# vinits5/learning3d

Hardware: AMD Instinct MI355X
Metric: clouds/sec DGCNN-fwd+Chamfer B=32 N=1024; kNN HBM GB/s vs peak at 1/2/4/8 GPU (higher is better)
Workload: dtype f32 (shared-MLP GEMMs as f16x2: fp32 operands carried as an fp16 high part + an fp16 residual (unscaled between the EdgeConv kernel and conv5, 2^12-scaled elsewhere), 3 fp16 MFMA products per fp32 product, f32 accumulate, fp32-level error -- tests bound it by 2x the fp32-MFMA kernel's own error agai

## Files before the change

learning3d_amd/csrc/chamfer.hip:

```cpp
#include "common.h"

#define CTILE 2048
#define CWAVES 4
#define CUNROLL 8
#ifndef CH_SMALL_TILE
#define CH_SMALL_TILE 0
#endif
#define CHAMFER_LL_BLOCKS 64
#define CHAMFER_LL_WS_BYTES (16 + CHAMFER_LL_BLOCKS * 16)

template <int QPL>
__global__ __launch_bounds__(64 * CWAVES) void chamfer_fwd_kernel(const float *__restrict__ xyz1,
                                                                  const float *__restrict__ xyz2, int N,
                                                                  int M, float *__restrict__ dist1,
                                                                  float *__restrict__ dist2,
                                                                  int32_t *__restrict__ idx1,
                                                                  int32_t *__restrict__ idx2)
{
    __shared__ float4 cand[CTILE];
    __shared__ float rbest[CWAVES][QPL][64];
    __shared__ int rbesti[CWAVES][QPL][64];
    const int tid = threadIdx.x, lane = tid & 63, wave = tid >> 6;
    const int b = blockIdx.y;
    const int dir = blockIdx.z;
    const float *qs = dir == 0 ? xyz1 : xyz2;
    const float *cs = dir == 0 ? xyz2 : xyz1;
    const int Nq = dir == 0 ? N : M;
    const int Nc = dir == 0 ? M : N;
    float *dout = dir == 0 ? dist1 : dist2;
    int32_t *iout = dir == 0 ? idx1 : idx2;
    const int q0 = blockIdx.x * (64 * QPL);
    if (q0 >= Nq) return;

    float qx[QPL], qy[QPL], qz[QPL], best[QPL];
    int besti[QPL];
#pragma unroll
    for (int u = 0; u < QPL; u++) {
        int q = min(q0 + u * 64 + lane, Nq - 1);
        const float *p = qs + ((size_t)b * Nq + q) * 3;
        qx[u] = p[0]; qy[u] = p[1]; qz[u] = p[2];
        best[u] = INFINITY; besti[u] = 0x7fffffff;
    }
    const float *cbase = cs + (size_t)b * Nc * 3;
    for (int c0 = 0; c0 < Nc; c0 += CTILE) {
        const int tn = min(CTILE, Nc - c0);
        __syncthreads();
        l3d_stage_points<8>(cbase + (size_t)c0 * 3, tn, tid, 64 * CWAVES, [&](int t, float x, float y, float z) { cand[t] = make_float4(x, y, z, 0.f); });
        __syncthreads();
        const int per = (tn + CWAVES - 1) / CWAVES;
        const int t0 = wave * per, t1 = min(tn, t0 + per);
        int t = t0;
        for (; t + CUNROLL <= t1; t += CUNROLL) {
            float4 c[CUNROLL];
#pragma unroll
            for (int v = 0; v < CUNROLL; v++) c[v] = cand[t + v];
#pragma unroll
            for (int v = 0; v < CUNROLL; v++)
#pragma unroll
                for (int u = 0; u < QPL; u++) {
                    const float dx = c[v].x - qx[u], dy = c[v].y - qy[u], dz = c[v].z - qz[u];
                    const float d = (dx * dx + dy * dy) + dz * dz;
                    const bool lt = d < best[u];
                    best[u] = lt ? d : best[u];
                    besti[u] = lt ? c0 + t + v : besti[u];
                }
        }
        for (; t < t1; t++) {
            const float4 c = cand[t];
#pragma unroll
            for (int u = 0; u < QPL; u++) {
                const float dx = c.x - qx[u], dy = c.y - qy[u], dz = c.z - qz[u];
                const float d = (dx * dx + dy * dy) + dz * dz;
                const bool lt = d < best[u];
                best[u] = lt ? d : best[u];
                besti[u] = lt ? c0 + t : besti[u];
            }
        }
    }
#pragma unroll
    for (int u = 0; u < QPL; u++) { rbest[wave][u][lane] = best[u]; rbesti[wave][u][lane] = besti[u]; }
    __syncthreads();
    if (wave == 0) {
#pragma unroll
        for (int u = 0; u < QPL; u++) {
            float bv = rbest[0][u][lane];
            int bi = rbesti[0][u][lane];
#pragma unroll
            for (int w = 1; w < CWAVES; w++) {
                const float ov = rbest[w][u][lane];
                const int oi = rbesti[w][u][lane];
                const bool take = ov < bv || (ov == bv && oi < bi);
                bv = take ? ov : bv;
                bi = take ? oi : bi;
            }
            const int q = q0 + u * 64 + lane;
            if (q < Nq) {
                dout[(size_t)b * Nq + q] = bv;
                iout[(size_t)b * Nq + q] = bi == 0x7fffffff ? 0 : bi;
            }
        }
    }
}

__device__ __forceinline__ void chamfer_loss_tail(double sq, unsigned *__restrict__ ws, double *__restrict__ partial,
                                                  float *__restrict__ loss, int N, int M)
{
    const int lane = threadIdx.x & 63;
    for (int off = 32; off > 0; off >>= 1) sq += __shfl_down(sq, off, 64);
    double *slots = (double *)(ws + 4);
    const unsigned per_dir = gridDim.x * gridDim.y, total = 2 * per_dir;
    const unsigned slot = (blockIdx.z * gridDim.y + blockIdx.y) * gridDim.x + blockIdx.x;
    unsigned ticket = 0;
    if (lane == 0) {
        __hip_atomic_store(&slots[slot], sq, __ATOMIC_RELAXED, __HIP_MEMORY_SCOPE_AGENT);
        asm volatile("s_waitcnt vmcnt(0)" ::: "memory");
        ticket = __hip_atomic_fetch_add(ws, 1u, __ATOMIC_RELAXED, __HIP_MEMORY_SCOPE_AGENT);
    }
    ticket = __builtin_amdgcn_readfirstlane(ticket);
    if (ticket != total - 1) return;
    double t[2];
#pragma unroll
    for (int z = 0; z < 2; z++) {
        double a = 0.0;
        for (unsigned i = lane; i < per_dir; i += 64) a += __hip_atomic_load(&slots[z * per_dir + i], __ATOMIC_RELAXED, __HIP_MEMORY_SCOPE_AGENT);
        for (int off = 32; off > 0; off >>= 1) a += __shfl_down(a, off, 64);
        t[z] = a;
    }
    if (lane == 0) {
        const double n1 = (double)gridDim.y * N, n2 = (double)gridDim.y * M;
        partial[0] = t[0]; partial[1] = t[1]; partial[2] = n1; partial[3] = n2;
        loss[0] = (float)((t[0] / n1 + t[1] / n2) / 2.0);
        __hip_atomic_store(ws, 0u, __ATOMIC_RELAXED, __HIP_MEMORY_SCOPE_AGENT);
    }
}


template <bool LOSS, int PTILE>
__global__ __launch_bounds__(64 * CWAVES) void chamfer_fwd_packed_kernel(const float *__restrict__ xyz1,
                                                                         const float *__restrict__ xyz2, int N, int M,
                                                                         float *__restrict__ dist1,
                                                                         float *__restrict__ dist2,
                                                                         int32_t *__restrict__ idx1,
                                                                         int32_t *__restrict__ idx2,
                                                                         unsigned *__restrict__ ws, double *__restrict__ partial,
                                                                         float *__restrict__ loss)
{
    typedef float f32x2 __attribute__((ext_vector_type(2)));
    __shared__ float4 cand[PTILE];
    __shared__ float rbest[CWAVES][2][64];
    __shared__ int rbesti[CWAVES][2][64];
    const int tid = threadIdx.x, lane = tid & 63, wave = tid >> 6;
    const int b = blockIdx.y;
    const int dir = blockIdx.z;
    const float *qs = dir == 0 ? xyz1 : xyz2;
    const float *cs = dir == 0 ? xyz2 : xyz1;
    const int Nq = dir == 0 ? N : M;
    const int Nc = dir == 0 ? M : N;
    float *dout = dir == 0 ? dist1 : dist2;
    int32_t *iout = dir == 0 ? idx1 : idx2;
    const int q0 = blockIdx.x * 128;
    if (!LOSS && q0 >= Nq) return;
    if (LOSS && q0 >= Nq) {
        if (wave == 0) chamfer_loss_tail(0.0, ws, partial, loss, N, M);
        return;
    }

    f32x2 qx, qy, qz;
    {
        const float *p0 = qs + ((size_t)b * Nq + min(q0 + lane, Nq - 1)) * 3;
        const float *p1 = qs + ((size_t)b * Nq + min(q0 + 64 + lane, Nq - 1)) * 3;
        qx = f32x2{p0[0], p1[0]}; qy = f32x2{p0[1], p1[1]}; qz = f32x2{p0[2], p1[2]};
    }
    float best0 = INFINITY, best1 = INFINITY;
    int base0 = 0x7fffffff, base1 = 0x7fffffff;
    const float *cbase = cs + (size_t)b * Nc * 3;
    for (int c0 = 0; c0 < Nc; c0 += PTILE) {
        const int tn = min(PTILE, Nc - c0);
        __syncthreads();
        {
            constexpr int NS = PTILE / (64 * CWAVES);
            float sx[NS], sy[NS], sz[NS];
#pragma unroll
            for (int i = 0; i < NS; i++) {
                const float *cp = cbase + (size_t)(c0 + min(tid + i * 64 * CWAVES, tn - 1)) * 3;
                sx[i] = cp[0]; sy[i] = cp[1]; sz[i] = cp[2];
            }
#pragma unroll
            for (int i = 0; i < NS; i++) {
                const int t = tid + i * 64 * CWAVES;
                if (t < tn) cand[t] = make_float4(sx[i], sy[i], sz[i], 0.f);
            }
        }
        __syncthreads();
        const int per = (tn + CWAVES - 1) / CWAVES;
        const int t0 = wave * per, t1 = min(tn, t0 + per);
        int t = t0;
        for (; t + 8 <= t1; t += 8) {
            float4 c[8];
#pragma unroll
            for (int v = 0; v < 8; v++) c[v] = cand[t + v];
            f32x2 d[8];
#pragma unroll
            for (int v = 0; v < 8; v++) {
                const f32x2 dx = f32x2{c[v].x, c[v].x} - qx, dy = f32x2{c[v].y, c[v].y} - qy, dz = f32x2{c[v].z, c[v].z} - qz;
                d[v] = (dx * dx + dy * dy) + dz * dz;
            }
            float m0 = fminf(fminf(d[0][0], d[1][0]), d[2][0]), m1 = fminf(fminf(d[0][1], d[1][1]), d[2][1]);
            m0 = fminf(fminf(m0, d[3][0]), d[4][0]); m1 = fminf(fminf(m1, d[3][1]), d[4][1]);
            m0 = fminf(fminf(m0, d[5][0]), d[6][0]); m1 = fminf(fminf(m1, d[5][1]), d[6][1]);
            m0 = fminf(m0, d[7][0]); m1 = fminf(m1, d[7][1]);
            const bool lt0 = m0 < best0, lt1 = m1 < best1;
            best0 = lt0 ? m0 : best0; base0 = lt0 ? c0 + t : base0;
            best1 = lt1 ? m1 : best1; base1 = lt1 ? c0 + t : base1;
        }
        for (; t < t1; t++) {
            const float4 c = cand[t];
            const f32x2 dx = f32x2{c.x, c.x} - qx, dy = f32x2{c.y, c.y} - qy, dz = f32x2{c.z, c.z} - qz;
            const f32x2 d = (dx * dx + dy * dy) + dz * dz;
            const bool lt0 = d[0] < best0, lt1 = d[1] < best1;
            best0 = lt0 ? d[0] : best0; base0 = lt0 ? c0 + t : base0;
            best1 = lt1 ? d[1] : best1; base1 = lt1 ? c0 + t : base1;
        }
    }
    int bi0 = base0, bi1 = base1;
    {
        bool f0 = base0 == 0x7fffffff, f1 = base1 == 0x7fffffff;
#pragma unroll
        for (int v = 0; v < 8; v++) {
            const int j0 = min(base0 == 0x7fffffff ? 0 : base0 + v, Nc - 1), j1 = min(base1 == 0x7fffffff ? 0 : base1 + v, Nc - 1);
            const float *pa = cbase + (size_t)j0 * 3, *pb = cbase + (size_t)j1 * 3;
            const f32x2 dx = f32x2{pa[0], pb[0]} - qx, dy = f32x2{pa[1], pb[1]} - qy, dz = f32x2{pa[2], pb[2]} - qz;
            const f32x2 d = (dx * dx + dy * dy) + dz * dz;
            if (!f0 && d[0] == best0) { bi0 = j0; f0 = true; }
            if (!f1 && d[1] == best1) { bi1 = j1; f1 = true; }
        }
    }
    rbest[wave][0][lane] = best0; rbesti[wave][0][lane] = bi0;
    rbest[wave][1][lane] = best1; rbesti[wave][1][lane] = bi1;
    __syncthreads();
    if (wave == 0) {
        double sq = 0.0;
#pragma unroll
        for (int u = 0; u < 2; u++) {
            float bv = rbest[0][u][lane];
            int bi = rbesti[0][u][lane];
#pragma unroll
            for (int w = 1; w < CWAVES; w++) {
                const float ov = rbest[w][u][lane];
                const int oi = rbesti[w][u][lane];
                const bool take = ov < bv || (ov == bv && oi < bi);
                bv = take ? ov : bv;
                bi = take ? oi : bi;
            }
            const int q = q0 + u * 64 + lane;
            if (q < Nq) {
                dout[(size_t)b * Nq + q] = bv;
                iout[(size_t)b * Nq + q] = bi == 0x7fffffff ? 0 : bi;
                if (LOSS) sq += (double)sqrtf(bv);
            }
        }
        if (LOSS) chamfer_loss_tail(sq, ws, partial, loss, N, M);
    }
}

int l3d_chamfer_forward_mfma(const float *xyz1, const float *xyz2, int B, int N, int M, float *dist1, float *dist2,
                             int32_t *idx1, int32_t *idx2, hipStream_t stream);

extern "C" int l3d_chamfer_forward_variant(const float *xyz1, const float *xyz2, int B, int N, int M,
                                           float *dist1, float *dist2, int32_t *idx1, int32_t *idx2,
                                           int variant, l3d_stream_t stream)
{
    L3D_REQUIRE(xyz1 && xyz2 && dist1 && dist2 && idx1 && idx2 && B > 0 && N > 0 && M > 0 && variant >= 0 && variant <= 3);
    L3D_REQUIRE(B <= 65535);
    const int l3d_chamfer_forward_mode = variant;
    const int mx = N > M ? N : M;
    if (variant == 3 || (variant == 1 && (long)N * M >= (1L << 24) && (long)2 * l3d_divup(mx, 512) * B >= 128))
        return l3d_chamfer_forward_mfma(xyz1, xyz2, B, N, M, dist1, dist2, idx1, idx2, (hipStream_t)stream);
    const long wgs2 = (long)l3d_divup(mx, 128) * B * 2;
    if (l3d_chamfer_forward_mode == 2 || (l3d_chamfer_forward_mode == 1 && wgs2 * CWAVES >= 1024)) {
        dim3 grid(l3d_divup(mx, 128), B, 2);
        if (mx <= 1024 && CH_SMALL_TILE)
            hipLaunchKernelGGL((chamfer_fwd_packed_kernel<false, 1024>), grid, dim3(64 * CWAVES), 0, (hipStream_t)stream, xyz1, xyz2, N, M,
                               dist1, dist2, idx1, idx2, (unsigned *)nullptr, (double *)nullptr, (float *)nullptr);
        else
            hipLaunchKernelGGL((chamfer_fwd_packed_kernel<false, CTILE>), grid, dim3(64 * CWAVES), 0, (hipStream_t)stream, xyz1, xyz2, N, M,
                               dist1, dist2, idx1, idx2, (unsigned *)nullptr, (double *)nullptr, (float *)nullptr);
    } else if (wgs2 * 2 >= 8192) {
        dim3 grid(l3d_divup(mx, 128), B, 2);
        hipLaunchKernelGGL(chamfer_fwd_kernel<2>, grid, dim3(64 * CWAVES), 0, (hipStream_t)stream, xyz1,
                           xyz2, N, M, dist1, dist2, idx1, idx2);
    } else {
        dim3 grid(l3d_divup(mx, 64), B, 2);
        hipLaunchKernelGGL(chamfer_fwd_kernel<1>, grid, dim3(64 * CWAVES), 0, (hipStream_t)stream, xyz1,
                           xyz2, N, M, dist1, dist2, idx1, idx2);
    }
    return l3d_check_launch();
}

extern "C" int l3d_chamfer_forward(const float *xyz1, const float *xyz2, int B, int N, int M,
                                   float *dist1, float *dist2, int32_t *idx1, int32_t *idx2,
                                   l3d_stream_t stream)
{
    return l3d_chamfer_forward_variant(xyz1, xyz2, B, N, M, dist1, dist2, idx1, idx2, 1, stream);
}

extern "C" int l3d_chamfer_loss_local_mb(const float *dist1, const float *dist2, int B, int N, int M, void *ws, double *partial, float *loss,
                                         l3d_stream_t stream);

extern "C" size_t l3d_chamfer_forward_loss_ws_bytes(int B, int N, int M)
{
    if (B <= 0 || N <= 0 || M <= 0) return 0;
    const size_t fused = 16 + (size_t)2 * B * l3d_divup(N > M ? N : M, 128) * sizeof(double);
    return fused > CHAMFER_LL_WS_BYTES ? fused : CHAMFER_LL_WS_BYTES;
}

extern "C" int l3d_chamfer_forward_loss(const float *xyz1, const float *xyz2, int B, int N, int M, float *dist1, float *dist2,
                                        int32_t *idx1, int32_t *idx2, void *ws, double *partial, float *loss, l3d_stream_t stream)
{
    L3D_REQUIRE(xyz1 && xyz2 && dist1 && dist2 && idx1 && idx2 && ws && partial && loss && B > 0 && N > 0 && M > 0);
    L3D_REQUIRE(B <= 65535);
    const int mx = N > M ? N : M;
    const long wgs2 = (long)l3d_divup(mx, 128) * B * 2;
    if ((long)N * M < (1L << 24) && wgs2 * CWAVES >= 1024) {
        dim3 grid(l3d_divup(mx, 128), B, 2);
        if (mx <= 1024 && CH_SMALL_TILE)
            hipLaunchKernelGGL((chamfer_fwd_packed_kernel<true, 1024>), grid, dim3(64 * CWAVES), 0, (hipStream_t)stream, xyz1, xyz2, N, M, dist1,
                               dist2, idx1, idx2, (unsigned *)ws, partial, loss);
        else
            hipLaunchKernelGGL((chamfer_fwd_packed_kernel<true, CTILE>), grid, dim3(64 * CWAVES), 0, (hipStream_t)stream, xyz1, xyz2, N, M, dist1,
                               dist2, idx1, idx2, (unsigned *)ws, partial, loss);
        return l3d_check_launch();
    }
    const int rc = l3d_chamfer_forward_variant(xyz1, xyz2, B, N, M, dist1, dist2, idx1, idx2, 1, stream);
    return rc ? rc : l3d_chamfer_loss_local_mb(dist1, dist2, B, N, M, ws, partial, loss, stream);
}

#define BTILE 4096
__global__ __launch_bounds__(64) void chamfer_bwd_kernel(const float *__restrict__ xyz1,
                                                         const float *__restrict__ xyz2, int N,
                                                         int M, const float *__restrict__ gd1,
                                                         const float *__restrict__ gd2,
                                                         const int32_t *__restrict__ idx1,
                                                         const int32_t *__restrict__ idx2,
                                                         float *__restrict__ g1,
                                                         float *__restrict__ g2)
{
    __shared__ int32_t sel[BTILE];
    const int lane = threadIdx.x;
    const int b = blockIdx.y;
    const int which = blockIdx.z;
    const float *A = which == 0 ? xyz1 : xyz2;
    const float *C = which == 0 ? xyz2 : xyz1;
    const int NA = which == 0 ? N : M;
    const int NC = which == 0 ? M : N;
    const float *gdA = which == 0 ? gd1 : gd2;
    const float *gdC = which == 0 ? gd2 : gd1;
    const int32_t *ia = which == 0 ? idx1 : idx2;
    const int32_t *ic = which == 0 ? idx2 : idx1;
    float *gout = which == 0 ? g1 : g2;
    if (blockIdx.x * 64 >= NA) return;
    const int i = blockIdx.x * 64 + lane;
    const bool valid = i < NA;
    const int iq = valid ? i : NA - 1;
    const float *ap = A + ((size_t)b * NA + iq) * 3;
    const float ax = ap[0], ay = ap[1], az = ap[2];
    const int j2 = ia[(size_t)b * NA + iq];
    const float *cp = C + ((size_t)b * NC + j2) * 3;
    const float g = gdA[(size_t)b * NA + iq] * 2;
    const float dxd = g * (ax - cp[0]), dyd = g * (ay - cp[1]), dzd = g * (az - cp[2]);
    float gx = 0.f, gy = 0.f, gz = 0.f;
    if (which == 0) { gx += dxd; gy += dyd; gz += dzd; }
    const int32_t *icb = ic + (size_t)b * NC;
    for (int c0 = 0; c0 < NC; c0 += BTILE) {
        const int tn = min(BTILE, NC - c0);
        __syncthreads();
        for (int t = lane; t < tn; t += 64) sel[t] = icb[c0 + t];
        __syncthreads();
        for (int g0 = 0; g0 < tn; g0 += 32) {
            unsigned mask = 0;
            const int gn = min(32, tn - g0);
            if (gn == 32) {
#pragma unroll
                for (int u = 0; u < 32; u++) mask |= sel[g0 + u] == iq ? (1u << u) : 0u;
            } else {
                for (int u = 0; u < gn; u++) mask |= sel[g0 + u] == iq ? (1u << u) : 0u;
            }
#pragma unroll 1
            while (__any(mask != 0)) {
                if (mask != 0) {
                    const int j = c0 + g0 + __builtin_ctz(mask);
                    mask &= mask - 1;
                    const float *pj = C + ((size_t)b * NC + j) * 3;
                    const float gj = gdC[(size_t)b * NC + j] * 2;
                    gx -= gj * (pj[0] - ax);
                    gy -= gj * (pj[1] - ay);
                    gz -= gj * (pj[2] - az);
                }
            }
        }
    }
    if (which == 1) { gx += dxd; gy += dyd; gz += dzd; }
    if (valid) {
        float *o = gout + ((size_t)b * NA + i) * 3;
        o[0] = gx; o[1] = gy; o[2] = gz;
    }
}

#define CB_SORT_MAX 32768
__global__ __launch_bounds__(1024) void chamfer_bwd_sorted_kernel(const float *__restrict__ xyz1,
                                                                  const float *__restrict__ xyz2, int N, int M,
                                                                  const float *__restrict__ gd1,
                                                                  const float *__restrict__ gd2,
                                                                  const int32_t *__restrict__ idx1,
                                                                  const int32_t *__restrict__ idx2,
                                                                  float *__restrict__ g1, float *__restrict__ g2,
                                                                  int P1, int P2, int shift1, int shift2)
{
    extern __shared__ uint32_t keys[];
    const int tid = threadIdx.x;
    const int b = blockIdx.x;
    const int which = blockIdx.y;
    const float *A = which == 0 ? xyz1 : xyz2;
    const float *C = which == 0 ? xyz2 : xyz1;
    const int NA = which == 0 ? N : M;
    const int NC = which == 0 ? M : N;
    const int P = which == 0 ? P2 : P1;
    const int shift = which == 0 ? shift2 : shift1;
    const float *gdA = (which == 0 ? gd1 : gd2) + (size_t)b * NA;
    const float *gdC = (which == 0 ? gd2 : gd1) + (size_t)b * NC;
    const int32_t *ia = (which == 0 ? idx1 : idx2) + (size_t)b * NA;
    const int32_t *ic = (which == 0 ? idx2 : idx1) + (size_t)b * NC;
    float *gout = (which == 0 ? g1 : g2) + (size_t)b * NA * 3;
    const float *Ab = A + (size_t)b * NA * 3, *Cb = C + (size_t)b * NC * 3;

    for (int t = tid; t < P; t += 1024) keys[t] = t < NC ? ((uint32_t)ic[t] << shift) | (uint32_t)t : 0xffffffffu;
    __syncthreads();
    for (int k = 2; k <= P; k <<= 1) {
        for (int j = k >> 1; j > 0; j >>= 1) {
            for (int t = tid; t < (P >> 1); t += 1024) {
                const int lo = ((t & ~(j - 1)) << 1) | (t & (j - 1)), hi = lo | j;
                const uint32_t x = keys[lo], y = keys[hi];
                const bool up = (lo & k) == 0;
                if ((x > y) == up) { keys[lo] = y; keys[hi] = x; }
            }
            __syncthreads();
        }
    }
    const uint32_t jmask = (1u << shift) - 1u;
    for (int i = tid; i < NA; i += 1024) {
        const float ax = Ab[i * 3], ay = Ab[i * 3 + 1], az = Ab[i * 3 + 2];
        const int j2 = ia[i];
        const float g = gdA[i] * 2;
        const float dxd = g * (ax - Cb[j2 * 3]), dyd = g * (ay - Cb[j2 * 3 + 1]), dzd = g * (az - Cb[j2 * 3 + 2]);
        float gx = 0.f, gy = 0.f, gz = 0.f;
        if (which == 0) { gx += dxd; gy += dyd; gz += dzd; }
        const uint32_t want = (uint32_t)i << shift;
        int lo = 0, hi = NC;
        while (lo < hi) {
            const int mid = (lo + hi) >> 1;
            if (keys[mid] < want) lo = mid + 1; else hi = mid;
        }
        for (int pos = lo; pos < NC; pos++) {
            const uint32_t key = keys[pos];
            if ((key >> shift) != (uint32_t)i) break;
            const int j = (int)(key & jmask);
            const float gj = gdC[j] * 2;
            gx -= gj * (Cb[j * 3] - ax);
            gy -= gj * (Cb[j * 3 + 1] - ay);
            gz -= gj * (Cb[j * 3 + 2] - az);
        }
        if (which == 1) { gx += dxd; gy += dyd; gz += dzd; }
        gout[i * 3] = gx; gout[i * 3 + 1] = gy; gout[i * 3 + 2] = gz;
    }
}

extern "C" int l3d_chamfer_backward_variant(const float *xyz1, const float *xyz2, int B, int N, int M,
                                            const float *graddist1, const float *graddist2,
                                            const int32_t *idx1, const int32_t *idx2, float *gradxyz1,
                                            float *gradxyz2, int variant, l3d_stream_t stream)
{
    L3D_REQUIRE(xyz1 && xyz2 && graddist1 && graddist2 && idx1 && idx2 && gradxyz1 && gradxyz2 &&
                B > 0 && N > 0 && M > 0 && variant >= 0 && variant <= 2);
    const int mx = N > M ? N : M;
    const bool sortable = mx <= CB_SORT_MAX;
    if (variant == 2 && !sortable) return L3D_ERR_UNSUPPORTED;
    if (variant != 0 && sortable) {
        int P1 = 2, P2 = 2, s1 = 1, s2 = 1;
        while (P1 < N) { P1 <<= 1; s1++; }
        while (P2 < M) { P2 <<= 1; s2++; }
        const size_t lds = sizeof(uint32_t) * (size_t)(P1 > P2 ? P1 : P2);
        hipLaunchKernelGGL(chamfer_bwd_sorted_kernel, dim3(B, 2), dim3(1024), lds, (hipStream_t)stream, xyz1, xyz2, N, M,
                           graddist1, graddist2, idx1, idx2, gradxyz1, gradxyz2, P1, P2, s1, s2);
        const int rc = l3d_check_launch();
        if (rc == L3D_OK || variant == 2) return rc;
    }
    dim3 grid(l3d_divup(mx, 64), B, 2);
    hipLaunchKernelGGL(chamfer_bwd_kernel, grid, dim3(64), 0, (hipStream_t)stream, xyz1, xyz2, N, M,
                       graddist1, graddist2, idx1, idx2, gradxyz1, gradxyz2);
    return l3d_check_launch();
}

extern "C" int l3d_chamfer_backward(const float *xyz1, const float *xyz2, int B, int N, int M,
                                    const float *graddist1, const float *graddist2,
                                    const int32_t *idx1, const int32_t *idx2, float *gradxyz1,
                                    float *gradxyz2, l3d_stream_t stream)
{
    return l3d_chamfer_backward_variant(xyz1, xyz2, B, N, M, graddist1, graddist2, idx1, idx2, gradxyz1, gradxyz2, 1, stream);
}

__global__ __launch_bounds__(1024) void sqrt_sum_kernel(const float *__restrict__ d1, size_t n1,
                                                        const float *__restrict__ d2, size_t n2,
                                                        double *__restrict__ partial)
{
    __shared__ double part[16];
    const int which = blockIdx.x;
    const float *d = which == 0 ? d1 : d2;
    const size_t n = which == 0 ? n1 : n2;
    double acc = 0.0;
    const size_t n4 = n >> 2;
    for (size_t i = threadIdx.x; i < n4; i += blockDim.x) {
        const float4 v = ((const float4 *)d)[i];
        acc += ((double)sqrtf(v.x) + (double)sqrtf(v.y)) + ((double)sqrtf(v.z) + (double)sqrtf(v.w));
    }
    for (size_t i = (n4 << 2) + threadIdx.x; i < n; i += blockDim.x) acc += (double)sqrtf(d[i]);
    for (int off = 32; off > 0; off >>= 1) acc += __shfl_down(acc, off, 64);
    if ((threadIdx.x & 63) == 0) part[threadIdx.x >> 6] = acc;
    __syncthreads();
    if (threadIdx.x == 0) {
        double t = 0.0;
        for (int w = 0; w < 16; w++) t += part[w];
        partial[which] = t;
        partial[2 + which] = (double)n;
    }
}

extern "C" int l3d_chamfer_partials(const float *dist1, const float *dist2, int B, int N, int M,
                                    double *partial, l3d_stream_t stream)
{
    L3D_REQUIRE(dist1 && dist2 && partial && B > 0 && N > 0 && M > 0);
    hipLaunchKernelGGL(sqrt_sum_kernel, dim3(2), dim3(1024), 0, (hipStream_t)stream, dist1,
                       (size_t)B * N, dist2, (size_t)B * M, partial);
    return l3d_check_launch();
}

__global__ __launch_bounds__(256) void chamfer_loss_local_mb_kernel(const float *__restrict__ d1, size_t n1,
                                                                    const float *__restrict__ d2, size_t n2,
                                                                    unsigned *__restrict__ ws, double *__restrict__ partial,
                                                                    float *__restrict__ loss)
{
    __shared__ double part[2][4];
    __shared__ bool last;
    double acc1 = 0.0, acc2 = 0.0;
    const size_t a4 = n1 >> 2, b4 = n2 >> 2, m4 = a4 > b4 ? a4 : b4;
    const size_t stride = (size_t)gridDim.x * 256;
    for (size_t i = (size_t)blockIdx.x * 256 + threadIdx.x; i < m4; i += stride) {
        if (i < a4) {
            const float4 v = ((const float4 *)d1)[i];
            acc1 += ((double)sqrtf(v.x) + (double)sqrtf(v.y)) + ((double)sqrtf(v.z) + (double)sqrtf(v.w));
        }
        if (i < b4) {
            const float4 v = ((const float4 *)d2)[i];
            acc2 += ((double)sqrtf(v.x) + (double)sqrtf(v.y)) + ((double)sqrtf(v.z) + (double)sqrtf(v.w));
        }
    }
    if (blockIdx.x == 0) {
        for (size_t i = (a4 << 2) + threadIdx.x; i < n1; i += 256) acc1 += (double)sqrtf(d1[i]);
        for (size_t i = (b4 << 2) + threadIdx.x; i < n2; i += 256) acc2 += (double)sqrtf(d2[i]);
    }
    for (int off = 32; off > 0; off >>= 1) { acc1 += __shfl_down(acc1, off, 64); acc2 += __shfl_down(acc2, off, 64); }
    if ((threadIdx.x & 63) == 0) { part[0][threadIdx.x >> 6] = acc1; part[1][threadIdx.x >> 6] = acc2; }
    __syncthreads();
    double *slots = (double *)(ws + 4);
    if (threadIdx.x == 0) {
        slots[2 * blockIdx.x] = (part[0][0] + part[0][1]) + (part[0][2] + part[0][3]);
        slots[2 * blockIdx.x + 1] = (part[1][0] + part[1][1]) + (part[1][2] + part[1][3]);
        __threadfence();
        last = atomicAdd(ws, 1u) == gridDim.x - 1;
    }
    __syncthreads();
    if (last && threadIdx.x < 64) {
        __threadfence();
        double t1 = 0.0, t2 = 0.0;
        if (threadIdx.x < gridDim.x) {
            t1 = __builtin_nontemporal_load(&slots[2 * threadIdx.x]);
            t2 = __builtin_nontemporal_load(&slots[2 * threadIdx.x + 1]);
        }
        for (int off = 32; off > 0; off >>= 1) { t1 += __shfl_down(t1, off, 64); t2 += __shfl_down(t2, off, 64); }
        if (threadIdx.x == 0) {
            partial[0] = t1; partial[1] = t2; partial[2] = (double)n1; partial[3] = (double)n2;
            loss[0] = (float)((t1 / (double)n1 + t2 / (double)n2) / 2.0);
            ws[0] = 0;
        }
    }
}

extern "C" size_t l3d_chamfer_loss_local_ws_bytes(void) { return CHAMFER_LL_WS_BYTES; }

extern "C" int l3d_chamfer_loss_local_mb(const float *dist1, const float *dist2, int B, int N, int M, void *ws, double *partial,
                                         float *loss, l3d_stream_t stream)
{
    L3D_REQUIRE(dist1 && dist2 && ws && partial && loss && B > 0 && N > 0 && M > 0);
    const size_t n1 = (size_t)B * N, n2 = (size_t)B * M, m4 = (n1 > n2 ? n1 : n2) >> 2;
    long blocks = l3d_divup((long)m4, 256);
    blocks = blocks < 1 ? 1 : (blocks > CHAMFER_LL_BLOCKS ? CHAMFER_LL_BLOCKS : blocks);
    hipLaunchKernelGGL(chamfer_loss_local_mb_kernel, dim3((unsigned)blocks), dim3(256), 0, (hipStream_t)stream, dist1, n1, dist2, n2,
                       (unsigned *)ws, partial, loss);
    return l3d_check_launch();
}


__global__ void chamfer_combine_kernel(const double *__restrict__ partials, int world,
                                       float *__restrict__ loss)
{
    if (threadIdx.x != 0) return;
    double s1 = 0, s2 = 0, n1 = 0, n2 = 0;
    for (int r = 0; r < world; r++) {
        s1 += partials[r * 4 + 0]; s2 += partials[r * 4 + 1];
        n1 += partials[r * 4 + 2]; n2 += partials[r * 4 + 3];
    }
    loss[0] = (float)((s1 / n1 + s2 / n2) / 2.0);
}

extern "C" int l3d_chamfer_combine(const double *partials, int world, float *loss, l3d_stream_t stream)
{
    L3D_REQUIRE(partials && loss && world > 0);
    hipLaunchKernelGGL(chamfer_combine_kernel, dim3(1), dim3(64), 0, (hipStream_t)stream, partials, world, loss);
    return l3d_check_launch();
}
```

Baseline: 124,600.

## Add multi-query-per-thread Chamfer forward path and optional one-WG loss reduction

Templates the packed Chamfer forward kernel on NP so each thread handles several query pairs against every candidate read from LDS. This cuts LDS candidate traffic and tile reloads per query, and is selected by default for mx<=2048 when enough workgroups remain. The price is fewer workgroups and more registers per thread. It also adds two macro-gated options that are off by default: a single-workgroup loss reduction and relaxed atomics in place of fences in the multi-block loss kernel.

```diff
diff --git a/learning3d_amd/csrc/chamfer.hip b/learning3d_amd/csrc/chamfer.hip
--- a/learning3d_amd/csrc/chamfer.hip
+++ b/learning3d_amd/csrc/chamfer.hip
@@ -5,6 +5,18 @@
 #define CUNROLL 8
 #ifndef CH_SMALL_TILE
 #define CH_SMALL_TILE 0
+#endif
+#ifndef CH_BLOCK_NP
+#define CH_BLOCK_NP 2
+#endif
+#ifndef CH_BLOCK_TILE
+#define CH_BLOCK_TILE CTILE
+#endif
+#ifndef CH_LOSS_ONE_WG
+#define CH_LOSS_ONE_WG 0
+#endif
+#ifndef CH_LL_FENCE
+#define CH_LL_FENCE 1
 #endif
 #define CHAMFER_LL_BLOCKS 64
 #define CHAMFER_LL_WS_BYTES (16 + CHAMFER_LL_BLOCKS * 16)
@@ -135,7 +147,7 @@
 }
 
 
-template <bool LOSS, int PTILE>
+template <bool LOSS, int PTILE, int NP>
 __global__ __launch_bounds__(64 * CWAVES) void chamfer_fwd_packed_kernel(const float *__restrict__ xyz1,
                                                                          const float *__restrict__ xyz2, int N, int M,
                                                                          float *__restrict__ dist1,
@@ -146,9 +158,11 @@
                                                                          float *__restrict__ loss)
 {
     typedef float f32x2 __attribute__((ext_vector_type(2)));
+    static_assert(!LOSS || NP == 1, "the loss tail's slots are per 128 queries");
+    constexpr int QW = 2 * NP;
     __shared__ float4 cand[PTILE];
-    __shared__ float rbest[CWAVES][2][64];
-    __shared__ int rbesti[CWAVES][2][64];
+    __shared__ float rbest[CWAVES][QW][64];
+    __shared__ int rbesti[CWAVES][QW][64];
     const int tid = threadIdx.x, lane = tid & 63, wave = tid >> 6;
     const int b = blockIdx.y;
     const int dir = blockIdx.z;
@@ -158,21 +172,24 @@
     const int Nc = dir == 0 ? M : N;
     float *dout = dir == 0 ? dist1 : dist2;
     int32_t *iout = dir == 0 ? idx1 : idx2;
-    const int q0 = blockIdx.x * 128;
+    const int q0 = blockIdx.x * (64 * QW);
     if (!LOSS && q0 >= Nq) return;
     if (LOSS && q0 >= Nq) {
         if (wave == 0) chamfer_loss_tail(0.0, ws, partial, loss, N, M);
         return;
     }
 
-    f32x2 qx, qy, qz;
-    {
-        const float *p0 = qs + ((size_t)b * Nq + min(q0 + lane, Nq - 1)) * 3;
-        const float *p1 = qs + ((size_t)b * Nq + min(q0 + 64 + lane, Nq - 1)) * 3;
-        qx = f32x2{p0[0], p1[0]}; qy = f32x2{p0[1], p1[1]}; qz = f32x2{p0[2], p1[2]};
-    }
-    float best0 = INFINITY, best1 = INFINITY;
-    int base0 = 0x7fffffff, base1 = 0x7fffffff;
+    f32x2 qx[NP], qy[NP], qz[NP];
+    float best0[NP], best1[NP];
+    int base0[NP], base1[NP];
+#pragma unroll
+    for (int p = 0; p < NP; p++) {
+        const float *p0 = qs + ((size_t)b * Nq + min(q0 + 128 * p + lane, Nq - 1)) * 3;
+        const float *p1 = qs + ((size_t)b * Nq + min(q0 + 128 * p + 64 + lane, Nq - 1)) * 3;
+        qx[p] = f32x2{p0[0], p1[0]}; qy[p] = f32x2{p0[1], p1[1]}; qz[p] = f32x2{p0[2], p1[2]};
+        best0[p] = INFINITY; best1[p] = INFINITY;
+        base0[p] = 0x7fffffff; base1[p] = 0x7fffffff;
+    }
     const float *cbase = cs + (size_t)b * Nc * 3;
     for (int c0 = 0; c0 < Nc; c0 += PTILE) {
         const int tn = min(PTILE, Nc - c0);
@@ -199,49 +216,57 @@
             float4 c[8];
 #pragma unroll
             for (int v = 0; v < 8; v++) c[v] = cand[t + v];
-            f32x2 d[8];
-#pragma unroll
-            for (int v = 0; v < 8; v++) {
-                const f32x2 dx = f32x2{c[v].x, c[v].x} - qx, dy = f32x2{c[v].y, c[v].y} - qy, dz = f32x2{c[v].z, c[v].z} - qz;
-                d[v] = (dx * dx + dy * dy) + dz * dz;
-            }
-            float m0 = fminf(fminf(d[0][0], d[1][0]), d[2][0]), m1 = fminf(fminf(d[0][1], d[1][1]), d[2][1]);
-            m0 = fminf(fminf(m0, d[3][0]), d[4][0]); m1 = fminf(fminf(m1, d[3][1]), d[4][1]);
-            m0 = fminf(fminf(m0, d[5][0]), d[6][0]); m1 = fminf(fminf(m1, d[5][1]), d[6][1]);
-            m0 = fminf(m0, d[7][0]); m1 = fminf(m1, d[7][1]);
-            const bool lt0 = m0 < best0, lt1 = m1 < best1;
-            best0 = lt0 ? m0 : best0; base0 = lt0 ? c0 + t : base0;
-            best1 = lt1 ? m1 : best1; base1 = lt1 ? c0 + t : base1;
+#pragma unroll
+            for (int p = 0; p < NP; p++) {
+                f32x2 d[8];
+#pragma unroll
+                for (int v = 0; v < 8; v++) {
+                    const f32x2 dx = f32x2{c[v].x, c[v].x} - qx[p], dy = f32x2{c[v].y, c[v].y} - qy[p], dz = f32x2{c[v].z, c[v].z} - qz[p];
+                    d[v] = (dx * dx + dy * dy) + dz * dz;
+                }
+                float m0 = fminf(fminf(d[0][0], d[1][0]), d[2][0]), m1 = fminf(fminf(d[0][1], d[1][1]), d[2][1]);
+                m0 = fminf(fminf(m0, d[3][0]), d[4][0]); m1 = fminf(fminf(m1, d[3][1]), d[4][1]);
+                m0 = fminf(fminf(m0, d[5][0]), d[6][0]); m1 = fminf(fminf(m1, d[5][1]), d[6][1]);
+                m0 = fminf(m0, d[7][0]); m1 = fminf(m1, d[7][1]);
+                const bool lt0 = m0 < best0[p], lt1 = m1 < best1[p];
+                best0[p] = lt0 ? m0 : best0[p]; base0[p] = lt0 ? c0 + t : base0[p];
+                best1[p] = lt1 ? m1 : best1[p]; base1[p] = lt1 ? c0 + t : base1[p];
+            }
         }
         for (; t < t1; t++) {
             const float4 c = cand[t];
-            const f32x2 dx = f32x2{c.x, c.x} - qx, dy = f32x2{c.y, c.y} - qy, dz = f32x2{c.z, c.z} - qz;
+#pragma unroll
+            for (int p = 0; p < NP; p++) {
+                const f32x2 dx = f32x2{c.x, c.x} - qx[p], dy = f32x2{c.y, c.y} - qy[p], dz = f32x2{c.z, c.z} - qz[p];
+                const f32x2 d = (dx * dx + dy * dy) + dz * dz;
+                const bool lt0 = d[0] < best0[p], lt1 = d[1] < best1[p];
+                best0[p] = lt0 ? d[0] : best0[p]; base0[p] = lt0 ? c0 + t : base0[p];
+                best1[p] = lt1 ? d[1] : best1[p]; base1[p] = lt1 ? c0 + t : base1[p];
+            }
+        }
+    }
+#pragma unroll
+    for (int p = 0; p < NP; p++) {
+        int bi0 = base0[p], bi1 = base1[p];
+        bool f0 = base0[p] == 0x7fffffff, f1 = base1[p] == 0x7fffffff;
+#pragma unroll
+        for (int v = 0; v < 8; v++) {
+            const int j0 = min(base0[p] == 0x7fffffff ? 0 : base0[p] + v, Nc - 1), j1 = min(base1[p] == 0x7fffffff ? 0 : base1[p] + v, Nc - 1);
+            const float *pa = cbase + (size_t)j0 * 3, *pb = cbase + (size_t)j1 * 3;
+            const f32x2 dx = f32x2{pa[0], pb[0]} - qx[p], dy = f32x2{pa[1], pb[1]} - qy[p], dz = f32x2{pa[2], pb[2]} - qz[p];
             const f32x2 d = (dx * dx + dy * dy) + dz * dz;
-            const bool lt0 = d[0] < best0, lt1 = d[1] < best1;
-            best0 = lt0 ? d[0] : best0; base0 = lt0 ? c0 + t : base0;
-            best1 = lt1 ? d[1] : best1; base1 = lt1 ? c0 + t : base1;
-        }
-    }
-    int bi0 = base0, bi1 = base1;
-    {
-        bool f0 = base0 == 0x7fffffff, f1 = base1 == 0x7fffffff;
-#pragma unroll
-        for (int v = 0; v < 8; v++) {
-            const int j0 = min(base0 == 0x7fffffff ? 0 : base0 + v, Nc - 1), j1 = min(base1 == 0x7fffffff ? 0 : base1 + v, Nc - 1);
-            const float *pa = cbase + (size_t)j0 * 3, *pb = cbase + (size_t)j1 * 3;
-            const f32x2 dx = f32x2{pa[0], pb[0]} - qx, dy = f32x2{pa[1], pb[1]} - qy, dz = f32x2{pa[2], pb[2]} - qz;
-            const f32x2 d = (dx * dx + dy * dy) + dz * dz;
-            if (!f0 && d[0] == best0) { bi0 = j0; f0 = true; }
-            if (!f1 && d[1] == best1) { bi1 = j1; f1 = true; }
-        }
-    }
-    rbest[wave][0][lane] = best0; rbesti[wave][0][lane] = bi0;
-    rbest[wave][1][lane] = best1; rbesti[wave][1][lane] = bi1;
+            if (!f0 && d[0] == best0[p]) { bi0 = j0; f0 = true; }
+            if (!f1 && d[1] == best1[p]) { bi1 = j1; f1 = true; }
+        }
+        rbest[wave][2 * p][lane] = best0[p]; rbesti[wave][2 * p][lane] = bi0;
+        rbest[wave][2 * p + 1][lane] = best1[p]; rbesti[wave][2 * p + 1][lane] = bi1;
+    }
     __syncthreads();
-    if (wave == 0) {
+    if (NP > 1 || wave == 0) {
         double sq = 0.0;
 #pragma unroll
-        for (int u = 0; u < 2; u++) {
+        for (int uu = 0; uu < (NP > 1 ? QW / CWAVES : QW); uu++) {
+            const int u = NP > 1 ? wave + uu * CWAVES : uu;
             float bv = rbest[0][u][lane];
             int bi = rbesti[0][u][lane];
 #pragma unroll
@@ -270,20 +295,27 @@
                                            float *dist1, float *dist2, int32_t *idx1, int32_t *idx2,
                                            int variant, l3d_stream_t stream)
 {
-    L3D_REQUIRE(xyz1 && xyz2 && dist1 && dist2 && idx1 && idx2 && B > 0 && N > 0 && M > 0 && variant >= 0 && variant <= 3);
+    L3D_REQUIRE(xyz1 && xyz2 && dist1 && dist2 && idx1 && idx2 && B > 0 && N > 0 && M > 0 && variant >= 0 && variant <= 4);
     L3D_REQUIRE(B <= 65535);
     const int l3d_chamfer_forward_mode = variant;
     const int mx = N > M ? N : M;
     if (variant == 3 || (variant == 1 && (long)N * M >= (1L << 24) && (long)2 * l3d_divup(mx, 512) * B >= 128))
         return l3d_chamfer_forward_mfma(xyz1, xyz2, B, N, M, dist1, dist2, idx1, idx2, (hipStream_t)stream);
+    const long wgsb = (long)l3d_divup(mx, 128 * CH_BLOCK_NP) * B * 2;
+    if (variant == 4 || (variant == 1 && mx <= 2048 && wgsb >= 256)) {
+        dim3 grid(l3d_divup(mx, 128 * CH_BLOCK_NP), B, 2);
+        hipLaunchKernelGGL((chamfer_fwd_packed_kernel<false, CH_BLOCK_TILE, CH_BLOCK_NP>), grid, dim3(64 * CWAVES), 0, (hipStream_t)stream, xyz1, xyz2,
+                           N, M, dist1, dist2, idx1, idx2, (unsigned *)nullptr, (double *)nullptr, (float *)nullptr);
+        return l3d_check_launch();
+    }
     const long wgs2 = (long)l3d_divup(mx, 128) * B * 2;
     if (l3d_chamfer_forward_mode == 2 || (l3d_chamfer_forward_mode == 1 && wgs2 * CWAVES >= 1024)) {
         dim3 grid(l3d_divup(mx, 128), B, 2);
         if (mx <= 1024 && CH_SMALL_TILE)
-            hipLaunchKernelGGL((chamfer_fwd_packed_kernel<false, 1024>), grid, dim3(64 * CWAVES), 0, (hipStream_t)stream, xyz1, xyz2, N, M,
+            hipLaunchKernelGGL((chamfer_fwd_packed_kernel<false, 1024, 1>), grid, dim3(64 * CWAVES), 0, (hipStream_t)stream, xyz1, xyz2, N, M,
                                dist1, dist2, idx1, idx2, (unsigned *)nullptr, (double *)nullptr, (float *)nullptr);
         else
-            hipLaunchKernelGGL((chamfer_fwd_packed_kernel<false, CTILE>), grid, dim3(64 * CWAVES), 0, (hipStream_t)stream, xyz1, xyz2, N, M,
+            hipLaunchKernelGGL((chamfer_fwd_packed_kernel<false, CTILE, 1>), grid, dim3(64 * CWAVES), 0, (hipStream_t)stream, xyz1, xyz2, N, M,
                                dist1, dist2, idx1, idx2, (unsigned *)nullptr, (double *)nullptr, (float *)nullptr);
     } else if (wgs2 * 2 >= 8192) {
         dim3 grid(l3d_divup(mx, 128), B, 2);
@@ -324,10 +356,10 @@
     if ((long)N * M < (1L << 24) && wgs2 * CWAVES >= 1024) {
         dim3 grid(l3d_divup(mx, 128), B, 2);
         if (mx <= 1024 && CH_SMALL_TILE)
-            hipLaunchKernelGGL((chamfer_fwd_packed_kernel<true, 1024>), grid, dim3(64 * CWAVES), 0, (hipStream_t)stream, xyz1, xyz2, N, M, dist1,
+            hipLaunchKernelGGL((chamfer_fwd_packed_kernel<true, 1024, 1>), grid, dim3(64 * CWAVES), 0, (hipStream_t)stream, xyz1, xyz2, N, M, dist1,
                                dist2, idx1, idx2, (unsigned *)ws, partial, loss);
         else
-            hipLaunchKernelGGL((chamfer_fwd_packed_kernel<true, CTILE>), grid, dim3(64 * CWAVES), 0, (hipStream_t)stream, xyz1, xyz2, N, M, dist1,
+            hipLaunchKernelGGL((chamfer_fwd_packed_kernel<true, CTILE, 1>), grid, dim3(64 * CWAVES), 0, (hipStream_t)stream, xyz1, xyz2, N, M, dist1,
                                dist2, idx1, idx2, (unsigned *)ws, partial, loss);
         return l3d_check_launch();
     }
@@ -572,27 +604,92 @@
     __syncthreads();
     double *slots = (double *)(ws + 4);
     if (threadIdx.x == 0) {
+#if CH_LL_FENCE
         slots[2 * blockIdx.x] = (part[0][0] + part[0][1]) + (part[0][2] + part[0][3]);
         slots[2 * blockIdx.x + 1] = (part[1][0] + part[1][1]) + (part[1][2] + part[1][3]);
         __threadfence();
         last = atomicAdd(ws, 1u) == gridDim.x - 1;
+#else
+        __hip_atomic_store(&slots[2 * blockIdx.x], (part[0][0] + part[0][1]) + (part[0][2] + part[0][3]), __ATOMIC_RELAXED, __HIP_MEMORY_SCOPE_AGENT);
+        __hip_atomic_store(&slots[2 * blockIdx.x + 1], (part[1][0] + part[1][1]) + (part[1][2] + part[1][3]), __ATOMIC_RELAXED, __HIP_MEMORY_SCOPE_AGENT);
+        asm volatile("s_waitcnt vmcnt(0)" ::: "memory");
+        last = __hip_atomic_fetch_add(ws, 1u, __ATOMIC_RELAXED, __HIP_MEMORY_SCOPE_AGENT) == gridDim.x - 1;
+#endif
     }
     __syncthreads();
     if (last && threadIdx.x < 64) {
+        double t1 = 0.0, t2 = 0.0;
+#if CH_LL_FENCE
         __threadfence();
-        double t1 = 0.0, t2 = 0.0;
         if (threadIdx.x < gridDim.x) {
             t1 = __builtin_nontemporal_load(&slots[2 * threadIdx.x]);
             t2 = __builtin_nontemporal_load(&slots[2 * threadIdx.x + 1]);
         }
+#else
+        if (threadIdx.x < gridDim.x) {
+            t1 = __hip_atomic_load(&slots[2 * threadIdx.x], __ATOMIC_RELAXED, __HIP_MEMORY_SCOPE_AGENT);
+            t2 = __hip_atomic_load(&slots[2 * threadIdx.x + 1], __ATOMIC_RELAXED, __HIP_MEMORY_SCOPE_AGENT);
+        }
+#endif
         for (int off = 32; off > 0; off >>= 1) { t1 += __shfl_down(t1, off, 64); t2 += __shfl_down(t2, off, 64); }
         if (threadIdx.x == 0) {
             partial[0] = t1; partial[1] = t2; partial[2] = (double)n1; partial[3] = (double)n2;
             loss[0] = (float)((t1 / (double)n1 + t2 / (double)n2) / 2.0);
+#if CH_LL_FENCE
             ws[0] = 0;
-        }
-    }
-}
+#else
+            __hip_atomic_store(ws, 0u, __ATOMIC_RELAXED, __HIP_MEMORY_SCOPE_AGENT);
+#endif
+        }
+    }
+}
+
+#if CH_LOSS_ONE_WG
+template <int NV>
+__global__ __launch_bounds__(1024) void chamfer_loss_local_one_kernel(const float *__restrict__ d1, size_t n1,
+                                                                      const float *__restrict__ d2, size_t n2,
+                                                                      double *__restrict__ partial, float *__restrict__ loss)
+{
+    __shared__ double part[2][16 * NV];
+    const int tid = threadIdx.x, lane = tid & 63, wave = tid >> 6;
+    const size_t a4 = n1 >> 2, b4 = n2 >> 2;
+    float4 v1[NV], v2[NV];
+#pragma unroll
+    for (int j = 0; j < NV; j++) {
+        const size_t i = (size_t)(j * 16 + wave) * 64 + lane;
+        v1[j] = ((const float4 *)d1)[i < a4 ? i : a4 - 1];
+        v2[j] = ((const float4 *)d2)[i < b4 ? i : b4 - 1];
+    }
+    const size_t r1 = (a4 << 2) + tid, r2 = (b4 << 2) + tid;
+    const float e1 = d1[r1 < n1 ? r1 : n1 - 1], e2 = d2[r2 < n2 ? r2 : n2 - 1];
+#pragma unroll
+    for (int j = 0; j < NV; j++) {
+        const size_t i = (size_t)(j * 16 + wave) * 64 + lane;
+        double acc1 = 0.0, acc2 = 0.0;
+        if (i < a4) acc1 += ((double)sqrtf(v1[j].x) + (double)sqrtf(v1[j].y)) + ((double)sqrtf(v1[j].z) + (double)sqrtf(v1[j].w));
+        if (i < b4) acc2 += ((double)sqrtf(v2[j].x) + (double)sqrtf(v2[j].y)) + ((double)sqrtf(v2[j].z) + (double)sqrtf(v2[j].w));
+        if (j == 0 && tid < 256) {
+            if (r1 < n1) acc1 += (double)sqrtf(e1);
+            if (r2 < n2) acc2 += (double)sqrtf(e2);
+        }
+        for (int off = 32; off > 0; off >>= 1) { acc1 += __shfl_down(acc1, off, 64); acc2 += __shfl_down(acc2, off, 64); }
+        if (lane == 0) { part[0][j * 16 + wave] = acc1; part[1][j * 16 + wave] = acc2; }
+    }
+    __syncthreads();
+    if (tid < 64) {
+        double t1 = 0.0, t2 = 0.0;
+        if (tid < 4 * NV) {
+            t1 = (part[0][4 * tid] + part[0][4 * tid + 1]) + (part[0][4 * tid + 2] + part[0][4 * tid + 3]);
+            t2 = (part[1][4 * tid] + part[1][4 * tid + 1]) + (part[1][4 * tid + 2] + part[1][4 * tid + 3]);
+        }
+        for (int off = 32; off > 0; off >>= 1) { t1 += __shfl_down(t1, off, 64); t2 += __shfl_down(t2, off, 64); }
+        if (tid == 0) {
+            partial[0] = t1; partial[1] = t2; partial[2] = (double)n1; partial[3] = (double)n2;
+            loss[0] = (float)((t1 / (double)n1 + t2 / (double)n2) / 2.0);
+        }
+    }
+}
+#endif
 
 extern "C" size_t l3d_chamfer_loss_local_ws_bytes(void) { return CHAMFER_LL_WS_BYTES; }
 
@@ -603,6 +700,16 @@
     const size_t n1 = (size_t)B * N, n2 = (size_t)B * M, m4 = (n1 > n2 ? n1 : n2) >> 2;
     long blocks = l3d_divup((long)m4, 256);
     blocks = blocks < 1 ? 1 : (blocks > CHAMFER_LL_BLOCKS ? CHAMFER_LL_BLOCKS : blocks);
+    blocks = blocks < 1 ? 1 : (blocks > CHAMFER_LL_BLOCKS ? CHAMFER_LL_BLOCKS : blocks);
+#if CH_LOSS_ONE_WG
+    if (n1 >= 4 && n2 >= 4 && blocks <= 32) {
+        const int nv = (int)l3d_divup(blocks, 4);
+#define L3D_LL_ONE(NV) hipLaunchKernelGGL(chamfer_loss_local_one_kernel<NV>, dim3(1), dim3(1024), 0, (hipStream_t)stream, dist1, n1, dist2, n2, partial, loss)
+        if (nv <= 1) L3D_LL_ONE(1); else if (nv <= 2) L3D_LL_ONE(2); else if (nv <= 4) L3D_LL_ONE(4); else L3D_LL_ONE(8);
+#undef L3D_LL_ONE
+        return l3d_check_launch();
+    }
+#endif
     hipLaunchKernelGGL(chamfer_loss_local_mb_kernel, dim3((unsigned)blocks), dim3(256), 0, (hipStream_t)stream, dist1, n1, dist2, n2,
                        (unsigned *)ws, partial, loss);
     return l3d_check_launch();
```

Result: no change. 124,200 (-0.3%).
